# JosephCatrambone/aruco3

Measured on AMD Instinct MI355X. Metric: frames/sec at 1920x1080 ARUCO dict, higher is better.
Workload: dtype u8

## Files before the change

### aruco3_amd/_lib.py

```python
import ctypes as C
from pathlib import Path

import numpy as np

import os

_HERE = Path(__file__).resolve().parent
LIB_PATH = Path(os.environ["A3_HIP_LIB"]).resolve() if os.environ.get("A3_HIP_LIB") else _HERE / "libaruco3_hip.so"

OK, ERR_INVALID, ERR_HIP, ERR_CAPACITY, ERR_INTERNAL, ERR_NO_DEVICE, ERR_LIMIT = 0, -1, -2, -3, -4, -5, -6
FMT_RGB8, FMT_RGBA8, FMT_L8, FMT_BGRA8 = 0, 1, 2, 3
FMT_YUYV8, FMT_UYVY8 = 5, 6
MEM_HOST, MEM_DEVICE = 0, 1
PROFILE_OFF, PROFILE_STAGES, PROFILE_THRESHOLD_ONLY, PROFILE_THRESHOLD_SAMPLED = 0, 1, 2, 3
STAGE_THRESHOLD, STAGE_CONTOUR, STAGE_DECODE = 0, 1, 2
STEP_WHOLE, STEP_DECODE_DEFERRED, STEP_HELD_RELEASED_BY_LAST, STEP_HELD_RELEASED_EARLY, STEP_BURST_LAST, STEP_HELD = 0, 1, 2, 3, 4, 5
REFINE_NONE, REFINE_SUBPIX, REFINE_EDGES = 0, 1, 2
BOARD_NONE, BOARD_OK = 0, 1
BOARD_MAX_MARKERS = 1024
DIST_NONE, DIST_RATIONAL = 0, 1
DIST_FISHEYE = 3
CHARUCO_MAX_CORNERS = 2048
CHARUCO_NO_ADJ = 0xFFFFFFFF
CALIB_FIX_PRINCIPAL_POINT, CALIB_ZERO_TANGENT_DIST, CALIB_FIX_K3, CALIB_RATIONAL_MODEL, CALIB_USE_INTRINSIC_GUESS = 1, 2, 4, 8, 16
# ... 27 lines not shown
    "a3_candidate_count", "a3_download_candidates", "a3_download_homographies", "a3_estimate_pose", "a3_estimate_pose_normalized",
    "a3_find_nearest", "a3_calculate_tau", "a3_set_profiling", "a3_get_profile",
    "a3_contour_count", "a3_download_contours", "a3_detection_record_bytes", "a3_pack_detections",
    "a3_default_refine_config", "a3_set_corner_refinement", "a3_get_refined_corners", "a3_refine_corners",
    "a3_set_board", "a3_get_board_poses", "a3_estimate_board_pose",
    "a3_default_recover_config", "a3_set_board_recovery", "a3_get_board_recovery", "a3_get_recovered_counts", "a3_recover_markers",
    "a3_default_distortion", "a3_set_distortion", "a3_get_undistorted_corners", "a3_undistort_points",
    "a3_default_charuco_config", "a3_set_charuco", "a3_get_charuco_corners", "a3_get_charuco_poses", "a3_interpolate_charuco",
    "a3_calibrate_cameras", "a3_calibrate_fisheye_cameras", "a3_calibrate_rigs", "a3_calibrate_hand_eyes", "a3_build_marker_maps",
    "a3_default_rectify", "a3_rectify_frames", "a3_set_rectification", "a3_get_rectification",
    "a3_reduce_frames", "a3_set_reduction", "a3_get_reduction",
]
CAND_DTYPE = np.dtype([("start_key", "<u4"), ("xy", "<u2", (8,))])
PROJ_DTYPE = np.dtype([("inv", "<f4", (9,)), ("ok", "<i4")])
CONTOUR_DTYPE = np.dtype([("frame", "<u4"), ("start_key", "<u4"), ("point_base", "<u4"), ("n", "<u4")])
INTERNAL_SYMBOLS = ["a3_debug_set_overlap", "a3_debug_build_flags", "a3_debug_spin", "a3_debug_set_hold", "a3_debug_set_jump_rounds", "a3_debug_launch_threshold", "a3_debug_kernel_time", "a3_selftest_ieee", "a3_debug_clockwise", "a3_debug_rotate_bits", "a3_debug_discard_too_near", "a3_debug_inject_candidates", "a3_debug_sample_frames", "a3_debug_frame_candidates", "a3_debug_contour_quads"]


class A3Error(RuntimeError):
    def __init__(self, code, message):
        super().__init__(f"aruco3_hip error {code}: {message}")
        self.code = code


class Config(C.Structure):
    _fields_ = [
        ("threshold_window", C.c_uint32),
        ("contour_simplification_epsilon", C.c_double),
        ("min_side_length_factor", C.c_float),
        ("min_corner_separation_factor", C.c_float),
        ("homography_sample_size", C.c_uint32),
# ... 180 lines not shown


class RectifyInfo(C.Structure):
    _fields_ = [("tiles", C.c_uint32), ("path_tiles", C.c_uint32 * 4), ("reserved", C.c_uint32 * 3)]


class Stats(C.Structure):
    _fields_ = [("darts", C.c_uint64), ("contours_traced", C.c_uint64), ("contours_materialised", C.c_uint64),
                ("candidates_pre", C.c_uint64), ("candidates", C.c_uint64), ("markers", C.c_uint64),
                ("resolve_iterations", C.c_uint32), ("jump_rounds", C.c_uint32), ("chunks", C.c_uint32), ("stepping", C.c_uint32)]

    def as_dict(self):
        d = {k: int(getattr(self, k)) for k, _ in self._fields_}
        d["released_others"] = (d["stepping"] >> 8) & 0xFF
        d["reruns"] = (d["stepping"] >> 16) & 0xFF
        d["stepping"] = STEP_NAMES.get(d["stepping"] & 0xFF, d["stepping"] & 0xFF)
        return d


_lib = None


def load():
    global _lib
    if _lib is not None:
        return _lib
    try:
        import torch
    except ImportError:
        pass
# ... 49 lines not shown
    L.a3_synth_render.restype = C.c_int
    L.a3_synth_render.argtypes = [C.c_int, vp, vp, C.c_uint32, vp, C.c_uint32, C.c_uint32, C.c_uint32, C.c_int, C.c_float, C.c_float, C.c_int,
                                  vp, C.c_size_t, C.c_size_t]
    if hasattr(L, "a3_debug_set_overlap"):
        L.a3_debug_set_overlap.restype = C.c_int
        L.a3_debug_set_overlap.argtypes = [C.c_int]
    if hasattr(L, "a3_debug_launch_threshold"):
        L.a3_debug_launch_threshold.restype = C.c_int
        L.a3_debug_launch_threshold.argtypes = [vp, vp, C.c_int, C.c_uint32, C.c_uint32, C.c_uint32]
    if hasattr(L, "a3_debug_set_hold"):
        L.a3_debug_set_hold.restype = C.c_int
        L.a3_debug_set_hold.argtypes = [C.c_int]
    if hasattr(L, "a3_debug_set_jump_rounds"):
        L.a3_debug_set_jump_rounds.restype = C.c_int
        L.a3_debug_set_jump_rounds.argtypes = [C.c_int]
    if hasattr(L, "a3_debug_spin"):
        L.a3_debug_spin.restype = C.c_int
        L.a3_debug_spin.argtypes = [vp, C.c_int, C.c_int, C.c_int]
    if hasattr(L, "a3_debug_build_flags"):
        L.a3_debug_build_flags.restype = C.c_int
        L.a3_debug_build_flags.argtypes = []
    L.a3_debug_kernel_time.restype = C.c_int
    L.a3_debug_kernel_time.argtypes = [vp, C.c_int, C.c_int, C.c_int, C.POINTER(C.c_float)]
    L.a3_get_stats.restype = C.c_int
    L.a3_get_stats.argtypes = [vp, C.POINTER(Stats)]
    L.a3_download_grey.restype = C.c_int
    L.a3_download_grey.argtypes = [vp, C.c_uint32, u8p]
    L.a3_download_thresholded.restype = C.c_int
    L.a3_download_thresholded.argtypes = [vp, C.c_uint32, u8p]
    L.a3_candidate_count.restype = C.c_int
# ... 280 lines not shown
        check(load().a3_set_profiling(self.handle, int(mode)), self.handle)

    def profile(self, stage: int, reset: bool = False):
        ms, n = C.c_double(), C.c_uint64()
        check(load().a3_get_profile(self.handle, stage, C.byref(ms), C.byref(n), int(reset)), self.handle)
        return float(ms.value), int(n.value)

    def debug_kernel_time(self, kernel: int, dbg: int = 0, reps: int = 5) -> float:
        ms = C.c_float()
        check(load().a3_debug_kernel_time(self.handle, kernel, dbg, reps, C.byref(ms)), self.handle)
        return ms.value

    def stats(self) -> dict:
        s = Stats()
        check(load().a3_get_stats(self.handle, C.byref(s)), self.handle)
        return s.as_dict()

    def detect_batch(self, pixels_ptr: int, memory: int, fmt: int, width: int, height: int, row_stride: int, frame_stride: int, n_frames: int,
                     out_cap: int = 0):
        cap = out_cap or max(64 * n_frames, 64)
        out = np.empty(cap, dtype=MARKER_DTYPE)
        per = np.zeros(max(n_frames, 1), dtype=np.uint32)
        n = C.c_size_t()
        rc = load().a3_detect_batch(self.handle, C.c_void_p(pixels_ptr), memory, fmt, width, height, row_stride, frame_stride, n_frames,
                                    out.ctypes.data_as(C.c_void_p), cap, _p(per, C.c_uint32), C.byref(n))
        check(rc, self.handle)
        return out[: n.value], per[:n_frames]

    def submit(self, pixels_ptr: int, memory: int, fmt: int, width: int, height: int, row_stride: int, frame_stride: int, n_frames: int,
               out_cap: int = 0):
        self._pending = (out_cap or max(64 * n_frames, 64), n_frames)
# ... 432 lines not shown
```

### aruco3_amd/csrc/a3_api.hip

```cpp
#include <algorithm>
#include <atomic>
#include <cmath>
#include <chrono>
#include <cstddef>
#include <cstdio>
#include <cstring>
#include <mutex>
#include <string>
#include <vector>

#include "a3_common.h"
#include "a3_format.h"
#include "a3_internal.h"
#include "a3_launch.h"
#include "a3_readback.h"
#include "a3_rectify_check.h"
#include "a3_reduce_check.h"
#include "a3_solve_check.h"

using namespace a3;

namespace {

thread_local std::string g_create_error;
// ... 60 lines not shown
    uint32_t frames_W = 0, frames_H = 0;
    a3_rectify rect_r{};
    uint32_t reduce_f = 0;
    bool taps = false;
    bool sample_frames = false;
    int profiling = 0, profile_every = 1;
    int prof = 0;
    bool need_grey = false;
    bool grey_src = false;
    uint32_t max_cand = 0, patch_cap = 0, marker_cap = 0, guess = 0;
    bool active = false, device_plan = false;
    size_t n_chunks = 0;
    Readback rb;
    uint64_t chunk0_darts = 0;
    int rounds_max = 0;
    PixelSrc src{};
};

}

struct a3_ctx {
    int device = 0;
    hipStream_t own_stream = nullptr, stream = nullptr;
    hipEvent_t ev_in = nullptr;
    hipEvent_t ev_contours = nullptr, ev_k1 = nullptr, ev_k1_done = nullptr, ev_gate = nullptr;
    bool gates_declared = false;
    bool rest_held = false;
    int held_rc = 0;
    bool back_deferred = false;
    int back_rc = 0;
    bool allow_defer = false;
    int batch_mode = 0;
    std::atomic<uint32_t> stepping{0};
    uint32_t released_others = 0;
    uint32_t reruns = 0;
    a3_config cfg{};
    uint8_t num_bits = 0, tau = 0;
    uint32_t n_codes = 0, mark_size = 0;
    std::string err;

    uint64_t max_darts = kMaxDartsDefault;
    BatchHints hints;
    uint32_t dbg_nd = 0, dbg_frames = 0, dbg_chunks = 0;
    PixelSrc dbg_src{};
    std::vector<CandRec> inject;
    bool inject_armed = false;
    uint32_t inject_count = 0;
    Batch batch;
    bool pending_trivial = false;
// ... 138 lines not shown
    A3_HIP(ctx->t_cur.ensure(darts * 8));
    A3_HIP(ctx->t_next.ensure(darts * 8));
    A3_HIP(ctx->leader_list.ensure(leader_list_bytes((uint32_t)darts)));
    A3_HIP(ctx->leader_keep.ensure(leader_list_bytes((uint32_t)darts)));
    const size_t eslots = entry_slots((uint32_t)darts);
    A3_HIP(ctx->entry_list.ensure(eslots * 4));
    A3_HIP(ctx->es_a.ensure(eslots * entry_state_bytes()));
    A3_HIP(ctx->es_b.ensure(eslots * entry_state_bytes()));
    return A3_OK;
}

struct DeviceStreams { hipStream_t decode = nullptr, copy = nullptr; };
std::mutex g_streams_mu;
DeviceStreams g_dev_streams[64];
bool g_hold_rests = true;
std::atomic<int> g_jump_rounds_cap{0};
enum { kStreamCopy = 0, kStreamDecode = 1 };

hipError_t create_stream(hipStream_t* st) { return hipStreamCreateWithPriority(st, hipStreamNonBlocking, 0); }

hipError_t device_stream(int device, int kind, hipStream_t* out) {
    std::lock_guard<std::mutex> lk(g_streams_mu);
    DeviceStreams& ds = g_dev_streams[device & 63];
    hipStream_t& st = kind == kStreamDecode ? ds.decode : ds.copy;
    if (!st) {
        const hipError_t e = create_stream(&st);
        if (e != hipSuccess) { st = nullptr; return e; }
    }
    *out = st;
    return hipSuccess;
// ... 300 lines not shown
                                      .bits = ctx->bin.as<uint64_t>(), .hsum_tmp = big_window ? ctx->hsum.as<uint16_t>() : nullptr}));
    if (b.prof) A3_HIP(hipEventRecord(ctx->ev[1], st));
    if (!held) return A3_OK;
    A3_HIP(hipEventRecord(ctx->ev_k1_done, st));
    const uint64_t cap_d = device_plan_capacity(ctx->hints, ctx->max_darts, n, W, H);
    if (cap_d == 0) return fail(ctx, A3_ERR_INTERNAL, "a chain was held back for a batch that needs a host-side plan");
    return ensure_chain_buffers(ctx, st, b, cap_d);
}

ContourChunk contour_chunk(const a3_ctx* ctx) {
    ContourChunk c;
    c.W = (int)ctx->W; c.H = (int)ctx->H; c.batch_frames = ctx->frames;
    c.bits = ctx->bin.as<uint64_t>(); c.tile_darts = ctx->tile_darts.as<uint32_t>(); c.pix_base = ctx->pix_base.as<uint32_t>();
    c.d_rec = ctx->d_xy.as<uint64_t>(); c.d_succ = ctx->d_succ.as<uint32_t>();
    c.entry_list = ctx->entry_list.as<uint32_t>(); c.es_a = ctx->es_a.p; c.es_b = ctx->es_b.p; c.fin = ctx->fin.p;
    c.leader_count = ctx->head->leader_count; c.entry_count = ctx->head->entry_count;
    c.leader_list = ctx->leader_list.as<uint32_t>(); c.leader_keep = ctx->leader_keep.as<uint32_t>();
    c.t_cur = ctx->t_cur.as<uint64_t>(); c.t_next = ctx->t_next.as<uint64_t>();
    c.contours = ctx->contours.as<ContourRec>(); c.cyc_start_off = ctx->cyc_start_off.as<uint32_t>(); c.points = ctx->points.as<uint32_t>();
    c.max_contours = ctx->hints.max_contours; c.max_points = ctx->hints.max_points;
    c.cands = ctx->cands.as<CandRec>(); c.cand_count = ctx->cand_count;
    c.err_flags = &ctx->head->err_flags;
    return c;
}

int enqueue_chain(a3_ctx* ctx, Batch& b, bool defer_locked) {
    hipStream_t st = ctx->stream;
    const uint32_t n = b.n, W = b.W, H = b.H;
    const int rel_mode = defer_locked ? 0 : release_mode();
    const size_t npx = (size_t)W * H;
    const uint32_t minwh = W < H ? W : H;
// ... 77 lines not shown
        uint32_t* h_bases = reinterpret_cast<uint32_t*>((uint8_t*)ctx->pinned + (size_t)n * 8);
        for (size_t ci = 0; ci < chunks.size(); ci++) chunk_frame_bases(fd.data(), chunks[ci], (uint32_t)stride, h_bases + ci * stride);
        A3_HIP(hipMemcpyAsync(ctx->frame_base.p, h_bases, n_bases * 4, hipMemcpyHostToDevice, st));
    }
    ctx->stats.chunks = (uint32_t)chunks.size();

    ContourChunk cc = contour_chunk(ctx);
    cc.n_live = n_live;
    cc.resolve_iters = ctx->hints.resolve_full_ttl > 0 ? ctx->hints.resolve_iters_hint : 0;
    cc.inline_resolve_W = ctx->hints.resolve_full_ttl > 0 ? 0 : (int)W;
    cc.min_edge_length = min_edge_length;
    cc.eps_factor = ctx->cfg.contour_simplification_epsilon;
    cc.keep_all = b.taps;
    cc.max_cand = kMaxCand;
    int rounds_max = 0;
    for (size_t ci = 0; ci < chunks.size(); ci++) {
        const Chunk& c = chunks[ci];
        const uint32_t nd = (uint32_t)c.darts;
        if (nd == 0) continue;
        if (ci > 0) {
            A3_HIP(hipMemsetAsync(cc.leader_count, 0, sizeof(BatchScratch::leader_count) + sizeof(BatchScratch::entry_count), st));
            A3_HIP(hipMemsetAsync(ctx->frame_cursor, 0, (size_t)c.count * 4, st));
        }
        cc.first_frame = c.first; cc.n_frames = c.count; cc.n_darts = nd;
        cc.frame_base = ctx->frame_base.as<uint32_t>() + ci * (max_chunk_frames + 1);
        cc.ctr = ctx->counters + ci;
        A3_HIP(launch_dart_build(st, cc));
        const int rounds = chunk_rounds(c.max_frame_darts, ctx->hints.jump_rounds_hint, g_jump_rounds_cap.load(std::memory_order_relaxed));
        rounds_max = std::max(rounds_max, rounds);
        cc.max_rounds = rounds;
        cc.frame_entries = ctx->hints.entry_global_ttl > 0 ? nullptr : ctx->frame_cursor;
        const bool dense_graph = (uint64_t)nd * 10u >= (uint64_t)c.count * npx;
        cc.dead_count = (b.taps || !dense_graph) ? nullptr : ctx->head->dead_count;
        cc.phase = 1;
        A3_HIP(launch_rank_cycles(st, cc));
        if (rel_mode == 2) { if (int rc = release_waiting()) return rc; }
        ctx->dbg_nd = nd; ctx->dbg_frames = c.count; ctx->dbg_chunks = (uint32_t)chunks.size();
        cc.phase = 2;
        A3_HIP(launch_rank_cycles(st, cc));
        A3_HIP(launch_resolve(st, cc));
        A3_HIP(launch_select_scatter(st, cc));
        A3_HIP(launch_contour_quads(st, cc));
    }
    if (rel_mode != 0) { if (int rc = release_waiting()) return rc; }
    if (b.prof >= 2) A3_HIP(hipEventRecord(ctx->ev[2], st));

// ... 34 lines not shown
    hipStream_t st = ctx->stream;
    const size_t n_chunks = b.n_chunks;
    const uint32_t guess = b.guess, n = b.n;
    uint8_t* hp = (uint8_t*)ctx->pinned;
    Readback rb = b.rb;
    {
        std::lock_guard<std::mutex> lk(g_defer_mu);
        if (int rc = flush_deferred_locked(ctx, nullptr)) return rc;
        if (const int rc = ctx->back_rc) { ctx->back_rc = 0; return rc; }
    }
    A3_HIP(wait_event(ctx->ev[4], st));
    const BatchScratch& hs = *reinterpret_cast<const BatchScratch*>(hp);
    const DeviceCounters* hc = reinterpret_cast<const DeviceCounters*>(&hs + 1);
    const size_t slot_bytes = sizeof(CandRec) + 16 + 16 + 4 + decode_out_bytes() + proj_rec_bytes();
    const Verdict v = batch_verdict(hs, hc, {.n = n, .W = b.W, .H = b.H, .device_plan = b.device_plan, .n_chunks = n_chunks, .chunk0_darts = b.chunk0_darts,
                                             .rounds_max = b.rounds_max, .out_cap = out_cap, .lds_slots = frame_cand_lds_slots(), .slot_bytes = slot_bytes},
                                    ctx->hints);
    if (b.device_plan && !hs.plan.overflow) ctx->stats.darts = ctx->dbg_nd = v.darts;
    ctx->stats.contours_traced = v.contours_traced; ctx->stats.contours_materialised = v.contours_materialised;
    ctx->stats.jump_rounds = v.jump_rounds; ctx->stats.resolve_iterations = v.resolve_iterations;
    if (v.action == Verdict::Fail) return fail(ctx, v.code, v.message);
    if (v.action == Verdict::GrowCands) {
        const size_t had = ctx->cands.cap + ctx->pre_xy.cap + ctx->fin_xy.cap + ctx->work.cap + ctx->cand_big.cap + ctx->outs.cap + ctx->proj.cap;
        const size_t want = (size_t)n * v.next_cand * v.slot_bytes;
        size_t free_b = 0, total_b = 0;
        if (want > had && hipMemGetInfo(&free_b, &total_b) == hipSuccess && want - had > free_b)
            return fail(ctx, A3_ERR_LIMIT, "candidate tables of this batch do not fit the device (every frame gets the fullest frame's table): fewer frames per call");
        ctx->hints.max_cand = v.next_cand;
    }
    if (v.action != Verdict::Deliver) return 1;
    const uint32_t total = v.total, n_work = v.n_work, n_pre = v.n_pre;
    const uint32_t* hpf = reinterpret_cast<const uint32_t*>(hc + n_chunks);
    if (per_frame_count) memcpy(per_frame_count, hpf, (size_t)n * 4);
    uint32_t max_per_frame = 0;
    for (uint32_t f = 0; f < n; f++) max_per_frame = std::max(max_per_frame, hpf[f]);
// ... 423 lines not shown
    const int rc = stage_input(ctx, pixels, memory, fmt, width, height, &b.row_stride, &b.frame_stride, n_frames, &b.pixels);
    if (rc != A3_OK) return rc;
    b.frames = PixelSrc{b.pixels, b.row_stride, b.frame_stride, fmt}; b.frames_W = width; b.frames_H = height;
    b.plane = ctx->rect_on ? Batch::Plane::Rectified : ctx->reduction.factor ? Batch::Plane::Reduced : Batch::Plane::None;
    if (b.plane != Batch::Plane::None) {
        size_t w, h;
        if (b.plane == Batch::Plane::Rectified) { b.rect_r = ctx->rect; w = b.rect_r.dst.image_width; h = b.rect_r.dst.image_height; }
        else { b.reduce_f = ctx->reduction.factor; w = width / b.reduce_f; h = height / b.reduce_f; }
        A3_HIP(ctx->plane.ensure(w * h * n_frames));
        b.pixels = ctx->plane.as<uint8_t>(); b.fmt = A3_FMT_L8; b.W = (uint32_t)w; b.H = (uint32_t)h;
        b.row_stride = w; b.frame_stride = w * h;
    }
    if (b.board || b.charuco || b.recover) { if (int urc = upload_board(ctx)) return urc; }
    if (b.recover) { if (int urc = upload_recover_ids(ctx)) return urc; }
    if (b.charuco) { if (int urc = upload_charuco(ctx)) return urc; }
    ctx->hints.force_host_plan = false;
    ctx->reruns = 0; ctx->released_others = 0;
    return A3_OK;
}

static void finish_trivial(a3_ctx* ctx, uint32_t* per_frame_count) {
    const Batch& b = ctx->batch;
    if (per_frame_count && b.n) memset(per_frame_count, 0, (size_t)b.n * 4);
    for (int k = 0; k < kSideKinds; k++) {
        if (!kSides[k].kept) continue;
        ctx->side_h[k].assign(b.has(k) && kSides[k].per_frame ? b.n * kSides[k].rec : 0, 0);
        ctx->side_valid[k] = b.has(k);
    }
    ctx->h_charuco.clear(); ctx->charuco_valid = b.charuco;
}

static int run_batch_with_retries(a3_ctx* ctx, a3_marker* out, a3_pose* poses, size_t out_cap, uint32_t* per_frame_count, size_t* out_n) {
// ... 219 lines not shown
}

int a3_debug_set_hold(int on) {
    std::lock_guard<std::mutex> lk(g_defer_mu);
    if (!g_held.empty()) return A3_ERR_INVALID;
    g_hold_rests = on != 0;
    return A3_OK;
}

int a3_debug_set_jump_rounds(int rounds) {
    if (rounds < 0 || rounds > 32) return A3_ERR_INVALID;
    g_jump_rounds_cap.store(rounds, std::memory_order_relaxed);
    return A3_OK;
}

int a3_synth_render(int device, void* hip_stream, const a3_synth_frame* frames, uint32_t n_frames, const a3_synth_marker* markers,
                    uint32_t n_markers, uint32_t width, uint32_t height, int paper, float black, float white, int supersample,
                    void* out_rgb_device, size_t row_stride, size_t frame_stride) {
    if (!frames || !out_rgb_device || (n_markers && !markers) || supersample < 1 || supersample > 8) return A3_ERR_INVALID;
    if (n_frames == 0 || width == 0 || height == 0) return A3_OK;
    if (row_stride == 0) row_stride = (size_t)width * 3;
    if (frame_stride == 0) frame_stride = row_stride * height;
    if (row_stride < (size_t)width * 3 || frame_stride < row_stride * (height - 1) + (size_t)width * 3 || height > 65535 || n_frames > 65535)
        return A3_ERR_INVALID;
    for (uint32_t f = 0; f < n_frames; f++)
        if ((uint64_t)frames[f].first_marker + frames[f].n_markers > n_markers) return A3_ERR_INVALID;
    for (uint32_t m = 0; m < n_markers; m++)
        if (markers[m].n == 0 || markers[m].n > 11) return A3_ERR_INVALID;
    if (hipSetDevice(device) != hipSuccess) return A3_ERR_NO_DEVICE;
    hipStream_t st = reinterpret_cast<hipStream_t>(hip_stream);
// ... 2 lines not shown
    if (e == hipSuccess && n_markers) e = hipMalloc(&d_markers, sizeof(a3_synth_marker) * n_markers);
    if (e == hipSuccess) e = hipMemcpyAsync(d_frames, frames, sizeof(a3_synth_frame) * n_frames, hipMemcpyHostToDevice, st);
    if (e == hipSuccess && n_markers) e = hipMemcpyAsync(d_markers, markers, sizeof(a3_synth_marker) * n_markers, hipMemcpyHostToDevice, st);
    if (e == hipSuccess) e = launch_synth_render(st, {.frames = d_frames, .n_frames = n_frames, .markers = d_markers, .W = width, .H = height, .paper = paper,
                                                      .black = black, .white = white, .supersample = supersample,
                                                      .out = reinterpret_cast<uint8_t*>(out_rgb_device), .row_stride = row_stride, .frame_stride = frame_stride});
    if (e == hipSuccess) e = hipStreamSynchronize(st);
    if (d_frames) (void)hipFree(d_frames);
    if (d_markers) (void)hipFree(d_markers);
    return e == hipSuccess ? A3_OK : A3_ERR_HIP;
}

int a3_get_stats(const a3_ctx* ctx, a3_stats* stats) {
    if (!ctx || !stats) return A3_ERR_INVALID;
    *stats = ctx->stats;
    stats->stepping = ctx->stepping | (std::min(ctx->released_others, 255u) << 8) | (std::min(ctx->reruns, 255u) << 16);
    return A3_OK;
}

static int download_plane(a3_ctx* ctx, const DevBuf& buf, uint32_t frame, uint8_t* dst) {
    if (!ctx || !dst) return A3_ERR_INVALID;
    if (frame >= ctx->frames) return fail(ctx, A3_ERR_INVALID, "frame index outside the last batch");
    const size_t npx = (size_t)ctx->W * ctx->H;
    A3_HIP(hipSetDevice(ctx->device));
    if (int rcs_ = need_stream(ctx)) return rcs_;
    A3_HIP(hipMemcpy(dst, buf.as<uint8_t>() + npx * frame, npx, hipMemcpyDeviceToHost));
    return A3_OK;
}

int a3_download_grey(a3_ctx* ctx, uint32_t frame, uint8_t* dst) {
    if (!ctx) return A3_ERR_INVALID;
// ... 1139 lines not shown
```

### aruco3_amd/csrc/a3_batch_head.h

```cpp
#pragma once
#include <cstddef>
#include <cstdint>

#include "../../include/aruco3_hip.h"

namespace a3 {

template <typename T> constexpr T min_of(T a, T b) { return b < a ? b : a; }
template <typename T> constexpr T max_of(T a, T b) { return a < b ? b : a; }

constexpr uint32_t kMaxChunkFrames = 65536u;
constexpr int kResolveItersMax = 16;
constexpr uint32_t kLeaderShards = 16, kEntryShards = 16, kDeadShards = 16;

struct DeviceCounters {
    unsigned long long darts;
    unsigned long long points;
    unsigned int contours;
    unsigned int traced;
    unsigned int err_flags;
    unsigned int resolve_needed;
    unsigned int jump_changed[32];
    unsigned int resolve_changed[16];
    unsigned int entry_overflow;
    unsigned int pad[1];
};
static_assert(sizeof(DeviceCounters::resolve_changed) / sizeof(unsigned int) == kResolveItersMax, "one resolve_changed slot per pass");

constexpr unsigned kErrBrokenEvent = 1u,
                   kErrPointPool = 2u, kErrContourTable = 4u, kErrCandTable = 8u,
                   kErrResolve = 16u,
                   kErrMarkerCap = 32u,
                   kErrScatter = 64u;

struct PlanWords {
    uint32_t darts;
    uint32_t overflow;
    uint32_t max_frame_darts;
    uint32_t total_clamped;
};
struct BatchScratch {
    unsigned int work_count;
    unsigned int marker_total;
    unsigned int cand_pre_total;
    unsigned int pack_overflow;
    unsigned int err_flags;
    unsigned int cand_most;
    unsigned int unused6[2];
    PlanWords plan;
    unsigned int unused12[4];
    unsigned int leader_count[kLeaderShards];
    unsigned int entry_count[kEntryShards];
    unsigned int dead_count[kDeadShards];
};
static_assert(offsetof(BatchScratch, work_count) == 0 && offsetof(BatchScratch, marker_total) == 4 && offsetof(BatchScratch, cand_pre_total) == 8 &&
              offsetof(BatchScratch, pack_overflow) == 12 && offsetof(BatchScratch, err_flags) == 16 && offsetof(BatchScratch, cand_most) == 20 &&
              offsetof(BatchScratch, plan) == 32 && offsetof(PlanWords, darts) == 0 && offsetof(PlanWords, overflow) == 4 &&
              offsetof(PlanWords, max_frame_darts) == 8 && offsetof(PlanWords, total_clamped) == 12 && offsetof(BatchScratch, leader_count) == 64 &&
              offsetof(BatchScratch, entry_count) == 128 && offsetof(BatchScratch, dead_count) == 192 && sizeof(BatchScratch) == 256,
              "the scratch words' offsets are part of the read-back head");
static_assert(offsetof(BatchScratch, entry_count) == offsetof(BatchScratch, leader_count) + sizeof(BatchScratch::leader_count),
              "leader and entry counts are cleared by one memset");
constexpr unsigned kCandMostFromPre = (offsetof(BatchScratch, cand_most) - offsetof(BatchScratch, cand_pre_total)) / sizeof(unsigned int);

constexpr uint32_t kMaxCandDefault = 1024, kMaxCandLimit = A3_MAX_CANDIDATES_PER_FRAME;
static_assert(kMaxCandLimit == 65536, "a3_marker.candidate_index is a uint16_t");
constexpr uint32_t kMaxContoursDefault = 1u << 20;
constexpr uint64_t kMaxDartsDefault = 48ull << 20;
constexpr uint64_t kMaxPointsDefault = 64ull << 20;
constexpr uint64_t kHardMaxDarts = (1ull << 30) - (1ull << 16);
constexpr uint64_t kHardMaxPoints = 3ull << 30;

struct BatchHints {
    int jump_rounds_hint = 10, resolve_iters_hint = 4;
    int resolve_full_ttl = 0;
    int entry_global_ttl = 0;
    bool plan_valid = false, force_host_plan = false;
    uint32_t plan_n = 0, plan_W = 0, plan_H = 0;
    uint64_t plan_darts = 0;
    uint64_t max_points = kMaxPointsDefault;
    uint32_t max_contours = kMaxContoursDefault;
    uint32_t max_cand = kMaxCandDefault;
};

struct BatchFacts {
    uint32_t n, W, H; bool device_plan; size_t n_chunks; uint64_t chunk0_darts; int rounds_max; size_t out_cap; uint32_t lds_slots; size_t slot_bytes;
};
struct Verdict {
    enum Action { Deliver, Rerun, GrowCands, Fail } action = Deliver;
    int code = A3_OK; const char* message = nullptr;
    uint32_t next_cand = 0; size_t slot_bytes = 0;
    uint64_t darts = 0, contours_traced = 0, contours_materialised = 0; uint32_t jump_rounds = 0, resolve_iterations = 0;
    uint32_t total = 0, n_work = 0, n_pre = 0;
    uint32_t tap_contours = 0; uint64_t tap_points = 0;
};

inline Verdict batch_verdict(const BatchScratch& hs, const DeviceCounters* hc, const BatchFacts& f, BatchHints& h) {
    Verdict v;
    const auto rerun = [&v]() { v.action = Verdict::Rerun; return v; };
    const auto fail = [&v](int code, const char* message) { v.action = Verdict::Fail; v.code = code; v.message = message; return v; };
    if (f.device_plan) {
        if (hs.plan.overflow) { h.force_host_plan = true; return rerun(); }
        v.darts = hs.plan.darts;
        h.plan_darts = hs.plan.darts;
    } else {
        h.plan_valid = f.n_chunks == 1;
        h.plan_n = f.n; h.plan_W = f.W; h.plan_H = f.H;
        h.plan_darts = f.n_chunks == 1 ? f.chunk0_darts : 0;
    }
    unsigned int flags = hs.err_flags;
    for (unsigned int dead : hs.dead_count) v.contours_traced += dead;
    uint64_t need_points = 0; uint32_t need_contours = 0;
    bool jump_short = false, resolve_needed = false, entry_overflow = false;
    for (size_t ci = 0; ci < f.n_chunks; ci++) {
        const DeviceCounters& c = hc[ci];
        flags |= c.err_flags;
        resolve_needed |= c.resolve_needed != 0;
        entry_overflow |= c.entry_overflow != 0;
        need_points = max_of<uint64_t>(need_points, c.points);
        need_contours = max_of(need_contours, c.contours);
        v.contours_traced += c.traced;
        v.contours_materialised += c.contours;
        for (int r = 0; r < 32; r++) if (c.jump_changed[r]) v.jump_rounds = max_of<uint32_t>(v.jump_rounds, r + 1);
        uint32_t it = c.resolve_needed ? 1 : 0;
        for (int r = 0; r < kResolveItersMax - 1; r++) if (c.resolve_changed[r]) it = r + 2;
        v.resolve_iterations = max_of(v.resolve_iterations, it);
        if (f.rounds_max > 0 && f.rounds_max < 32 && c.jump_changed[f.rounds_max - 1] != 0) jump_short = true;
    }
    if (entry_overflow) { h.entry_global_ttl = 64; h.jump_rounds_hint = max_of(h.jump_rounds_hint, 12); return rerun(); }
    if (h.entry_global_ttl > 0) h.entry_global_ttl--;
    if (jump_short && h.jump_rounds_hint < 32) { h.jump_rounds_hint = 32; return rerun(); }
    if (resolve_needed) {
        const bool ran = h.resolve_full_ttl > 0;
        h.resolve_full_ttl = 64;
        if (!ran) return rerun();
    } else if (h.resolve_full_ttl > 0) h.resolve_full_ttl--;
    if ((flags & kErrResolve) && h.resolve_iters_hint < kResolveItersMax) { h.resolve_iters_hint = kResolveItersMax; return rerun(); }
    h.jump_rounds_hint = max_of(4, min_of(32, (int)v.jump_rounds + 2));
    if (flags & (kErrPointPool | kErrContourTable)) {
        if (need_points > h.max_points) h.max_points = min_of<uint64_t>(kHardMaxPoints, max_of(need_points, h.max_points * 2));
        if (need_contours > h.max_contours) h.max_contours = max_of(need_contours, h.max_contours * 2);
        return rerun();
    }
    if (flags & kErrBrokenEvent) return fail(A3_ERR_INTERNAL, "contour graph: a start event lies on an open chain");
// ... 91 lines not shown
```

### aruco3_amd/csrc/a3_internal.h

```cpp
#ifndef ARUCO3_HIP_INTERNAL_H
#define ARUCO3_HIP_INTERNAL_H

#include "../../include/aruco3_hip.h"

#ifdef __cplusplus
extern "C" {
#endif

int  a3_debug_kernel_time(a3_ctx *ctx, int kernel, int dbg, int reps, float *avg_ms);

int  a3_debug_set_overlap(int mode);

int  a3_debug_spin(void *hip_stream, int workgroups, int threads, int usec);

int  a3_debug_set_hold(int on);

int  a3_debug_set_jump_rounds(int rounds);

int  a3_debug_launch_threshold(a3_ctx *ctx, const void *pixels_device, int fmt, uint32_t width, uint32_t height, uint32_t n_frames);

int  a3_debug_build_flags(void);

int  a3_selftest_ieee(a3_ctx *ctx, const double *a, const double *b, size_t n, double *sqrt_a, double *a_div_b,
                      float *sqrtf_a, float *a_divf_b);

int  a3_debug_clockwise(a3_ctx *ctx, const int32_t *quads_xy, size_t n, int32_t *out_xy);
int  a3_debug_rotate_bits(a3_ctx *ctx, const uint8_t *bits, uint32_t n, uint32_t times, uint8_t *out);
int  a3_debug_inject_candidates(a3_ctx *ctx, const uint32_t *quads_xy, size_t n);
int  a3_debug_sample_frames(a3_ctx *ctx, int enabled);
int  a3_debug_discard_too_near(a3_ctx *ctx, const uint32_t *quads_xy, size_t n, float min_distance, uint32_t *out_xy, size_t *n_out);

typedef struct { uint32_t start_key; uint16_t xy[8]; } a3_debug_cand;
// ... 16 lines not shown
```

### aruco3_amd/csrc/a3_launch.h

```cpp
#pragma once

#include "a3_common.h"

namespace a3 {

struct ThresholdLaunch {
    const uint8_t* pixels = nullptr; int fmt = 0; size_t row_stride = 0, frame_stride = 0; int W = 0, H = 0; uint32_t n = 0, radius = 0;
    uint8_t* grey = nullptr; uint64_t* bits = nullptr; uint16_t* hsum_tmp = nullptr;
};
hipError_t launch_grey_threshold(hipStream_t st, const ThresholdLaunch& t);
bool threshold_writes_grey_plane(uint32_t radius);
hipError_t launch_k1_r1(hipStream_t st, const ThresholdLaunch& t);
hipError_t launch_k1_r2(hipStream_t st, const ThresholdLaunch& t);
bool ring_kernel_applies(uint32_t radius);
hipError_t launch_ring_threshold(hipStream_t st, const ThresholdLaunch& t);

size_t tile_darts_bytes(uint32_t W, uint32_t H, uint32_t n_frames);
struct DartCountLaunch {
    const uint64_t* bits = nullptr; int W = 0, H = 0; uint32_t first_frame = 0, n_frames = 0; unsigned long long* frame_darts = nullptr;
    uint32_t* tile_darts = nullptr; uint64_t plan_cap = 0; uint32_t* frame_base = nullptr; PlanWords* plan = nullptr; void* zero_p = nullptr;
    size_t zero_bytes = 0;
};
hipError_t launch_dart_count(hipStream_t st, const DartCountLaunch& d);
hipError_t launch_zero(hipStream_t st, void* p, size_t bytes);

size_t entry_state_bytes();
size_t fin_state_bytes();
size_t entry_slots(uint32_t n_darts);
size_t leader_list_bytes(uint32_t n_darts);

struct ContourChunk {
    uint32_t first_frame = 0, n_frames = 0, n_darts = 0; const uint32_t* frame_base = nullptr; DeviceCounters* ctr = nullptr;
    int max_rounds = 0;
    uint32_t* frame_entries = nullptr;
    unsigned int* dead_count = nullptr;
    int W = 0, H = 0;
    uint32_t batch_frames = 0;
    const uint64_t* bits = nullptr; const uint32_t* tile_darts = nullptr;
    const uint32_t* n_live = nullptr;
    uint32_t* pix_base = nullptr; uint64_t* d_rec = nullptr; uint32_t* d_succ = nullptr; uint32_t* entry_list = nullptr;
    unsigned int* entry_count = nullptr, * leader_count = nullptr;
    void* es_a = nullptr, * es_b = nullptr;
    void* fin = nullptr;
    uint32_t* leader_list = nullptr, * leader_keep = nullptr; uint64_t* t_cur = nullptr, * t_next = nullptr;
    int resolve_iters = 0;
    int inline_resolve_W = 0;
    uint32_t min_edge_length = 0; double eps_factor = 0.0; ContourRec* contours = nullptr; uint32_t* cyc_start_off = nullptr;
    uint32_t* points = nullptr; uint32_t max_contours = 0; uint64_t max_points = 0;
    bool keep_all = false;
// ... 167 lines not shown
```

### aruco3_amd/csrc/k_contours.hip

```cpp
#include <algorithm>
#include <cmath>

#include "a3_common.h"
#include "a3_launch.h"


namespace a3 {

constexpr int kFinB = 8;
constexpr int kScatB = 1;

struct Nb8 { uint64_t c; uint64_t n[8]; };

__device__ __forceinline__ uint64_t ldw(const uint64_t* __restrict__ img, int wpr, int H, int j, int y) {
    return (y >= 0 && y < H && j >= 0 && j < wpr) ? img[(size_t)y * wpr + j] : 0ull;
}

__device__ __forceinline__ void pdart_words(const Nb8& nb, uint64_t p[8]) {
#pragma unroll
    for (int k = 0; k < 8; k++) {
        uint64_t m = nb.c & nb.n[k] & ~nb.n[(k + 7) & 7];
        if ((k & 1) == 0) m &= ~nb.n[(k + 6) & 7];
        p[k] = m;
    }
// ... 800 lines not shown
        const uint32_t excl = block_excl_scan_256((uint32_t)__popc(lmask), s_lw, &total);
        if (total) {
            const uint32_t shard = blockIdx.x & (kLeaderShards - 1);
            if (threadIdx.x == 0) s_lbase = atomicAdd(&leader_count[shard], total);
            __syncthreads();
            uint32_t slot = s_lbase + excl;
            while (lmask) {
                const int u = __ffs(lmask) - 1;
                lmask &= lmask - 1;
                leader_list[(size_t)shard * leader_cap + slot++] = lo + threadIdx.x + (uint32_t)u * 256u;
            }
        }
    }
}

constexpr uint32_t kEntryLdsCap = 2048;
__global__ __launch_bounds__(256) void k_entry_frame(const uint32_t* __restrict__ entry_list, const uint32_t* __restrict__ frame_entries,
                                                     const uint32_t* __restrict__ frame_base, const FinState* __restrict__ fin,
                                                     const uint64_t* __restrict__ d_rec, int W,
                                                     EntryState* __restrict__ es, DeviceCounters* __restrict__ ctr,
                                                     uint32_t* __restrict__ leader_list ,
                                                     unsigned int* __restrict__ leader_count , uint32_t leader_cap) {
    struct __attribute__((aligned(16))) Rec { uint64_t key; uint32_t ptr; uint32_t off; };
    __shared__ Rec s_rec[kEntryLdsCap];
    __shared__ uint32_t s_dist[kEntryLdsCap];
    const uint32_t f = blockIdx.x;
    const uint32_t cnt = frame_entries[f], base = frame_base[f];
    if (cnt == 0) return;
    if (cnt > kEntryLdsCap) { if (threadIdx.x == 0) ctr->entry_overflow = 1u; return; }
    constexpr int PER = kEntryLdsCap / 256;
    uint64_t nk[PER]; uint32_t np[PER], no[PER], nd[PER];
    uint32_t m0[PER];
    constexpr int EB = 4;
    static_assert(PER % EB == 0, "whole batches");
#pragma unroll
    for (int u0 = 0; u0 < PER; u0 += EB) {
        if ((uint32_t)u0 * 256u >= cnt) break;
        uint32_t e[EB];
        FinState l[EB];
        uint64_t mr[EB];
#pragma unroll
        for (int u = 0; u < EB; u++) e[u] = entry_list[base + min(threadIdx.x + 256u * (uint32_t)(u0 + u), cnt - 1u)];
#pragma unroll
        for (int u = 0; u < EB; u++) l[u] = fin[e[u]];
#pragma unroll
        for (int u = 0; u < EB; u++) mr[u] = d_rec[entry_min_dart(e[u], l[u])];
#pragma unroll
        for (int u = 0; u < EB; u++) asm volatile("" : "+v"(mr[u]), "+v"(l[u].leader), "+v"(l[u].w));
#pragma unroll
        for (int u = 0; u < EB; u++) {
            const uint32_t i = threadIdx.x + 256u * (uint32_t)(u0 + u);
            const EntryState s0 = entry_start(e[u], l[u], mr[u], W, base + i);
            nk[u0 + u] = s0.key; no[u0 + u] = s0.off; nd[u0 + u] = s0.dist; np[u0 + u] = s0.ptr - base; m0[u0 + u] = (uint32_t)s0.key;
            if (i < cnt) { s_rec[i] = Rec{nk[u0 + u], np[u0 + u], no[u0 + u]}; s_dist[i] = nd[u0 + u]; }
        }
    }
    __syncthreads();
    for (int round = 0; round < 12; round++) {
        int changed = 0;
#pragma unroll
        for (int u = 0; u < PER; u++) {
            const uint32_t i = threadIdx.x + u * 256;
            if (i < cnt) {
                const uint32_t t = np[u] < cnt ? np[u] : i;
                const Rec w = s_rec[t];
                const uint32_t wd = s_dist[t];
                if (w.key < nk[u]) { nk[u] = w.key; no[u] = nd[u] + w.off; changed = 1; }
                nd[u] += wd;
                np[u] = w.ptr;
            }
        }
        const int any = __syncthreads_or(changed);
#pragma unroll
// ... 674 lines not shown
                               entry_list, entry_count, ecap, frame_base, frame_entries, n_live, dbg, min_edge_length, dead_count, trust_natural,
                               ll, leader_count, lcap);
        else if (frame_entries)
            hipLaunchKernelGGL((k_local_contract<kLTFrame, true>), dim3((n_darts + kLTFrame - 1) / kLTFrame), dim3(256), 0, st, n_darts, W, d_rec, d_succ, fin,
                               entry_list, entry_count, ecap, frame_base, frame_entries, n_live, dbg, min_edge_length, dead_count, trust_natural,
                               ll, leader_count, lcap);
        else
            hipLaunchKernelGGL((k_local_contract<kLT, true>), dim3((n_darts + kLT - 1) / kLT), dim3(256), 0, st, n_darts, W, d_rec, d_succ, fin,
                               entry_list, entry_count, ecap, frame_base, frame_entries, n_live, dbg, min_edge_length, dead_count, trust_natural,
                               ll, leader_count, lcap);
    }
    if (dbg || phase == 1) return hipGetLastError();
    EntryState* a = reinterpret_cast<EntryState*>(c.es_a);
    EntryState* b = reinterpret_cast<EntryState*>(c.es_b);
    if (frame_entries) {
        hipLaunchKernelGGL(k_entry_frame, dim3(n_frames), dim3(256), 0, st, entry_list, frame_entries, frame_base, fin, d_rec, W, a, ctr,
                           ll, leader_count, lcap);
        if (no_finalize) return hipGetLastError();
        const int fin_blocks = std::max(blocks_for(n_darts, 256, kFinBlocks), (int)(((uint64_t)n_darts + 256ull * 32 - 1) / (256ull * 32)));
        hipLaunchKernelGGL(k_jump_finalize, dim3(fin_blocks), dim3(256), 0, st, n_darts, a, fin,
                           leader_list, leader_count, leader_shard_cap(n_darts), n_live, ctr);
        return hipGetLastError();
    }
    const dim3 grid(blocks_for(n_darts / 16 + 1, 256, 1024)), block(256);
    hipLaunchKernelGGL(k_entry_init, grid, block, 0, st, entry_list, entry_count, fin, d_rec, W, a, ecap);
    for (int r = 0; r < c.max_rounds; r++) {
        hipLaunchKernelGGL(k_entry_jump, grid, block, 0, st, a, b, entry_count, ecap, r, ctr);
        EntryState* t = a; a = b; b = t;
    }
    const int fin_blocks = std::max(blocks_for(n_darts, 256, kFinBlocks), (int)(((uint64_t)n_darts + 256ull * 32 - 1) / (256ull * 32)));
    hipLaunchKernelGGL(k_jump_finalize, dim3(fin_blocks), block, 0, st, n_darts, a, fin,
                       leader_list, leader_count, leader_shard_cap(n_darts), n_live, ctr);
// ... 58 lines not shown
```

Before: 374,400.

## Template per-frame entry kernel on adaptive LDS capacity with rerun on overflow

The per-frame entry pointer-jumping kernel is templated on its LDS capacity (512, 1024 or 2048 entries). The host picks the capacity from a hint that tracks the largest per-frame entry count seen, and reruns the batch at a larger capacity when a frame does not fit. Smaller capacities use less LDS and fewer registers per thread, and need fewer jump rounds (10 or 11 instead of 12), which should raise occupancy and cut work. The cost is an extra atomicMax per block, added host hint logic, and possible full-batch reruns when entry counts grow past the chosen cap.

```diff
diff --git a/aruco3_amd/_lib.py b/aruco3_amd/_lib.py
--- a/aruco3_amd/_lib.py
+++ b/aruco3_amd/_lib.py
@@ -65,7 +65,7 @@
 CAND_DTYPE = np.dtype([("start_key", "<u4"), ("xy", "<u2", (8,))])
 PROJ_DTYPE = np.dtype([("inv", "<f4", (9,)), ("ok", "<i4")])
 CONTOUR_DTYPE = np.dtype([("frame", "<u4"), ("start_key", "<u4"), ("point_base", "<u4"), ("n", "<u4")])
-INTERNAL_SYMBOLS = ["a3_debug_set_overlap", "a3_debug_build_flags", "a3_debug_spin", "a3_debug_set_hold", "a3_debug_set_jump_rounds", "a3_debug_launch_threshold", "a3_debug_kernel_time", "a3_selftest_ieee", "a3_debug_clockwise", "a3_debug_rotate_bits", "a3_debug_discard_too_near", "a3_debug_inject_candidates", "a3_debug_sample_frames", "a3_debug_frame_candidates", "a3_debug_contour_quads"]
+INTERNAL_SYMBOLS = ["a3_debug_set_overlap", "a3_debug_build_flags", "a3_debug_spin", "a3_debug_set_hold", "a3_debug_set_jump_rounds", "a3_debug_set_entry_cap", "a3_debug_entry_info", "a3_debug_launch_threshold", "a3_debug_kernel_time", "a3_selftest_ieee", "a3_debug_clockwise", "a3_debug_rotate_bits", "a3_debug_discard_too_near", "a3_debug_inject_candidates", "a3_debug_sample_frames", "a3_debug_frame_candidates", "a3_debug_contour_quads"]
 
 
 class A3Error(RuntimeError):
@@ -276,6 +276,7 @@
         d = {k: int(getattr(self, k)) for k, _ in self._fields_}
         d["released_others"] = (d["stepping"] >> 8) & 0xFF
         d["reruns"] = (d["stepping"] >> 16) & 0xFF
+        d["entry_cap"] = ((d["stepping"] >> 24) & 0xFF) * 256
         d["stepping"] = STEP_NAMES.get(d["stepping"] & 0xFF, d["stepping"] & 0xFF)
         return d
 
@@ -355,6 +356,11 @@
     if hasattr(L, "a3_debug_set_jump_rounds"):
         L.a3_debug_set_jump_rounds.restype = C.c_int
         L.a3_debug_set_jump_rounds.argtypes = [C.c_int]
+    if hasattr(L, "a3_debug_set_entry_cap"):
+        L.a3_debug_set_entry_cap.restype = C.c_int
+        L.a3_debug_set_entry_cap.argtypes = [C.c_uint32]
+        L.a3_debug_entry_info.restype = C.c_int
+        L.a3_debug_entry_info.argtypes = [vp, C.POINTER(C.c_uint32), C.POINTER(C.c_uint32)]
     if hasattr(L, "a3_debug_spin"):
         L.a3_debug_spin.restype = C.c_int
         L.a3_debug_spin.argtypes = [vp, C.c_int, C.c_int, C.c_int]
@@ -665,7 +671,12 @@
     def stats(self) -> dict:
         s = Stats()
         check(load().a3_get_stats(self.handle, C.byref(s)), self.handle)
-        return s.as_dict()
+        d = s.as_dict()
+        if hasattr(load(), "a3_debug_entry_info"):
+            most, short = C.c_uint32(0), C.c_uint32(0)
+            check(load().a3_debug_entry_info(self.handle, C.byref(most), C.byref(short)), self.handle)
+            d["entry_most"], d["entry_cap_reruns"] = most.value, short.value
+        return d
 
     def detect_batch(self, pixels_ptr: int, memory: int, fmt: int, width: int, height: int, row_stride: int, frame_stride: int, n_frames: int,
                      out_cap: int = 0):
diff --git a/aruco3_amd/csrc/a3_api.hip b/aruco3_amd/csrc/a3_api.hip
--- a/aruco3_amd/csrc/a3_api.hip
+++ b/aruco3_amd/csrc/a3_api.hip
@@ -98,6 +98,7 @@
     Readback rb;
     uint64_t chunk0_darts = 0;
     int rounds_max = 0;
+    uint32_t entry_cap = 0;
     PixelSrc src{};
 };
 
@@ -117,6 +118,7 @@
     int batch_mode = 0;
     std::atomic<uint32_t> stepping{0};
     uint32_t released_others = 0;
+    uint32_t entry_cap = 0, entry_most = 0, entry_cap_reruns = 0;
     uint32_t reruns = 0;
     a3_config cfg{};
     uint8_t num_bits = 0, tau = 0;
@@ -285,6 +287,7 @@
 std::mutex g_streams_mu;
 DeviceStreams g_dev_streams[64];
 bool g_hold_rests = true;
+std::atomic<uint32_t> g_entry_cap_force{0};
 std::atomic<int> g_jump_rounds_cap{0};
 enum { kStreamCopy = 0, kStreamDecode = 1 };
 
@@ -615,7 +618,7 @@
     c.bits = ctx->bin.as<uint64_t>(); c.tile_darts = ctx->tile_darts.as<uint32_t>(); c.pix_base = ctx->pix_base.as<uint32_t>();
     c.d_rec = ctx->d_xy.as<uint64_t>(); c.d_succ = ctx->d_succ.as<uint32_t>();
     c.entry_list = ctx->entry_list.as<uint32_t>(); c.es_a = ctx->es_a.p; c.es_b = ctx->es_b.p; c.fin = ctx->fin.p;
-    c.leader_count = ctx->head->leader_count; c.entry_count = ctx->head->entry_count;
+    c.leader_count = ctx->head->leader_count; c.entry_count = ctx->head->entry_count; c.entry_most = &ctx->head->entry_most;
     c.leader_list = ctx->leader_list.as<uint32_t>(); c.leader_keep = ctx->leader_keep.as<uint32_t>();
     c.t_cur = ctx->t_cur.as<uint64_t>(); c.t_next = ctx->t_next.as<uint64_t>();
     c.contours = ctx->contours.as<ContourRec>(); c.cyc_start_off = ctx->cyc_start_off.as<uint32_t>(); c.points = ctx->points.as<uint32_t>();
@@ -723,6 +726,9 @@
     cc.keep_all = b.taps;
     cc.max_cand = kMaxCand;
     int rounds_max = 0;
+    const uint32_t entry_force = ctx->hints.entry_cap_retry ? 0u : g_entry_cap_force.load(std::memory_order_relaxed);
+    cc.entry_cap = entry_force ? entry_force : entry_cap_of(ctx->hints.entry_most_hint);
+    b.entry_cap = 0;
     for (size_t ci = 0; ci < chunks.size(); ci++) {
         const Chunk& c = chunks[ci];
         const uint32_t nd = (uint32_t)c.darts;
@@ -739,6 +745,7 @@
         rounds_max = std::max(rounds_max, rounds);
         cc.max_rounds = rounds;
         cc.frame_entries = ctx->hints.entry_global_ttl > 0 ? nullptr : ctx->frame_cursor;
+        if (cc.frame_entries) b.entry_cap = cc.entry_cap;
         const bool dense_graph = (uint64_t)nd * 10u >= (uint64_t)c.count * npx;
         cc.dead_count = (b.taps || !dense_graph) ? nullptr : ctx->head->dead_count;
         cc.phase = 1;
@@ -803,11 +810,13 @@
     const DeviceCounters* hc = reinterpret_cast<const DeviceCounters*>(&hs + 1);
     const size_t slot_bytes = sizeof(CandRec) + 16 + 16 + 4 + decode_out_bytes() + proj_rec_bytes();
     const Verdict v = batch_verdict(hs, hc, {.n = n, .W = b.W, .H = b.H, .device_plan = b.device_plan, .n_chunks = n_chunks, .chunk0_darts = b.chunk0_darts,
-                                             .rounds_max = b.rounds_max, .out_cap = out_cap, .lds_slots = frame_cand_lds_slots(), .slot_bytes = slot_bytes},
+                                             .rounds_max = b.rounds_max, .out_cap = out_cap, .lds_slots = frame_cand_lds_slots(), .slot_bytes = slot_bytes, .entry_cap = b.entry_cap},
                                     ctx->hints);
     if (b.device_plan && !hs.plan.overflow) ctx->stats.darts = ctx->dbg_nd = v.darts;
     ctx->stats.contours_traced = v.contours_traced; ctx->stats.contours_materialised = v.contours_materialised;
     ctx->stats.jump_rounds = v.jump_rounds; ctx->stats.resolve_iterations = v.resolve_iterations;
+    ctx->entry_cap = b.entry_cap; ctx->entry_most = std::max(ctx->entry_most, v.entry_most);
+    if (v.entry_cap_short) ctx->entry_cap_reruns++;
     if (v.action == Verdict::Fail) return fail(ctx, v.code, v.message);
     if (v.action == Verdict::GrowCands) {
         const size_t had = ctx->cands.cap + ctx->pre_xy.cap + ctx->fin_xy.cap + ctx->work.cap + ctx->cand_big.cap + ctx->outs.cap + ctx->proj.cap;
@@ -1261,8 +1270,8 @@
     if (b.board || b.charuco || b.recover) { if (int urc = upload_board(ctx)) return urc; }
     if (b.recover) { if (int urc = upload_recover_ids(ctx)) return urc; }
     if (b.charuco) { if (int urc = upload_charuco(ctx)) return urc; }
-    ctx->hints.force_host_plan = false;
-    ctx->reruns = 0; ctx->released_others = 0;
+    ctx->hints.force_host_plan = false; ctx->hints.entry_cap_retry = false;
+    ctx->reruns = 0; ctx->released_others = 0; ctx->entry_cap_reruns = 0; ctx->entry_most = 0;
     return A3_OK;
 }
 
@@ -1512,6 +1521,18 @@
     return A3_OK;
 }
 
+int a3_debug_set_entry_cap(uint32_t cap) {
+    if (cap != 0 && cap != 512 && cap != 1024 && cap != 2048) return A3_ERR_INVALID;
+    g_entry_cap_force.store(cap, std::memory_order_relaxed);
+    return A3_OK;
+}
+
+int a3_debug_entry_info(const a3_ctx* ctx, uint32_t* most, uint32_t* cap_reruns) {
+    if (!ctx || !most || !cap_reruns) return A3_ERR_INVALID;
+    *most = ctx->entry_most; *cap_reruns = ctx->entry_cap_reruns;
+    return A3_OK;
+}
+
 int a3_synth_render(int device, void* hip_stream, const a3_synth_frame* frames, uint32_t n_frames, const a3_synth_marker* markers,
                     uint32_t n_markers, uint32_t width, uint32_t height, int paper, float black, float white, int supersample,
                     void* out_rgb_device, size_t row_stride, size_t frame_stride) {
@@ -1544,7 +1565,7 @@
 int a3_get_stats(const a3_ctx* ctx, a3_stats* stats) {
     if (!ctx || !stats) return A3_ERR_INVALID;
     *stats = ctx->stats;
-    stats->stepping = ctx->stepping | (std::min(ctx->released_others, 255u) << 8) | (std::min(ctx->reruns, 255u) << 16);
+    stats->stepping = ctx->stepping | (std::min(ctx->released_others, 255u) << 8) | (std::min(ctx->reruns, 255u) << 16) | ((ctx->entry_cap / 256u) << 24);
     return A3_OK;
 }
 
diff --git a/aruco3_amd/csrc/a3_batch_head.h b/aruco3_amd/csrc/a3_batch_head.h
--- a/aruco3_amd/csrc/a3_batch_head.h
+++ b/aruco3_amd/csrc/a3_batch_head.h
@@ -25,6 +25,7 @@
     unsigned int entry_overflow;
     unsigned int pad[1];
 };
+constexpr unsigned kEntryOverflow = 1u, kEntryCapShort = 2u;
 static_assert(sizeof(DeviceCounters::resolve_changed) / sizeof(unsigned int) == kResolveItersMax, "one resolve_changed slot per pass");
 
 constexpr unsigned kErrBrokenEvent = 1u,
@@ -46,7 +47,8 @@
     unsigned int pack_overflow;
     unsigned int err_flags;
     unsigned int cand_most;
-    unsigned int unused6[2];
+    unsigned int entry_most;
+    unsigned int unused7[1];
     PlanWords plan;
     unsigned int unused12[4];
     unsigned int leader_count[kLeaderShards];
@@ -54,7 +56,7 @@
     unsigned int dead_count[kDeadShards];
 };
 static_assert(offsetof(BatchScratch, work_count) == 0 && offsetof(BatchScratch, marker_total) == 4 && offsetof(BatchScratch, cand_pre_total) == 8 &&
-              offsetof(BatchScratch, pack_overflow) == 12 && offsetof(BatchScratch, err_flags) == 16 && offsetof(BatchScratch, cand_most) == 20 &&
+              offsetof(BatchScratch, pack_overflow) == 12 && offsetof(BatchScratch, err_flags) == 16 && offsetof(BatchScratch, cand_most) == 20 && offsetof(BatchScratch, entry_most) == 24 &&
               offsetof(BatchScratch, plan) == 32 && offsetof(PlanWords, darts) == 0 && offsetof(PlanWords, overflow) == 4 &&
               offsetof(PlanWords, max_frame_darts) == 8 && offsetof(PlanWords, total_clamped) == 12 && offsetof(BatchScratch, leader_count) == 64 &&
               offsetof(BatchScratch, entry_count) == 128 && offsetof(BatchScratch, dead_count) == 192 && sizeof(BatchScratch) == 256,
@@ -75,6 +77,8 @@
     int jump_rounds_hint = 10, resolve_iters_hint = 4;
     int resolve_full_ttl = 0;
     int entry_global_ttl = 0;
+    uint32_t entry_most_hint = 0;
+    bool entry_cap_retry = false;
     bool plan_valid = false, force_host_plan = false;
     uint32_t plan_n = 0, plan_W = 0, plan_H = 0;
     uint64_t plan_darts = 0;
@@ -83,8 +87,21 @@
     uint32_t max_cand = kMaxCandDefault;
 };
 
+constexpr uint32_t kEntryCapMin = 512, kEntryCapMax = 2048;
+inline uint32_t entry_cap_of(uint32_t hint) { return hint == 0 ? kEntryCapMax : hint <= 512 ? 512u : hint <= 1024 ? 1024u : kEntryCapMax; }
+inline uint32_t entry_hint_follow(uint32_t hint, uint32_t most) {
+    const uint32_t want = max_of(kEntryCapMin, min_of<uint32_t>(kEntryCapMax, most <= kEntryCapMax / 2 ? most * 2u : kEntryCapMax));
+    if (hint == 0) return want;
+    hint = max_of(kEntryCapMin, min_of(kEntryCapMax, hint));
+    return want >= hint ? want : max_of(want, hint - hint / 8u);
+}
+inline uint32_t entry_hint_grow(uint32_t cap, uint32_t most) {
+    return max_of(min_of(kEntryCapMax, max_of(cap, kEntryCapMin / 2) * 2u), entry_hint_follow(kEntryCapMin, most));
+}
+
 struct BatchFacts {
     uint32_t n, W, H; bool device_plan; size_t n_chunks; uint64_t chunk0_darts; int rounds_max; size_t out_cap; uint32_t lds_slots; size_t slot_bytes;
+    uint32_t entry_cap = 0;
 };
 struct Verdict {
     enum Action { Deliver, Rerun, GrowCands, Fail } action = Deliver;
@@ -93,6 +110,8 @@
     uint64_t darts = 0, contours_traced = 0, contours_materialised = 0; uint32_t jump_rounds = 0, resolve_iterations = 0;
     uint32_t total = 0, n_work = 0, n_pre = 0;
     uint32_t tap_contours = 0; uint64_t tap_points = 0;
+    uint32_t entry_most = 0;
+    bool entry_cap_short = false;
 };
 
 inline Verdict batch_verdict(const BatchScratch& hs, const DeviceCounters* hc, const BatchFacts& f, BatchHints& h) {
@@ -111,12 +130,13 @@
     unsigned int flags = hs.err_flags;
     for (unsigned int dead : hs.dead_count) v.contours_traced += dead;
     uint64_t need_points = 0; uint32_t need_contours = 0;
-    bool jump_short = false, resolve_needed = false, entry_overflow = false;
+    bool jump_short = false, resolve_needed = false, entry_overflow = false, entry_cap_short = false;
     for (size_t ci = 0; ci < f.n_chunks; ci++) {
         const DeviceCounters& c = hc[ci];
         flags |= c.err_flags;
         resolve_needed |= c.resolve_needed != 0;
-        entry_overflow |= c.entry_overflow != 0;
+        entry_overflow |= (c.entry_overflow & ~kEntryCapShort) != 0;
+        entry_cap_short |= (c.entry_overflow & kEntryCapShort) != 0;
         need_points = max_of<uint64_t>(need_points, c.points);
         need_contours = max_of(need_contours, c.contours);
         v.contours_traced += c.traced;
@@ -127,7 +147,17 @@
         v.resolve_iterations = max_of(v.resolve_iterations, it);
         if (f.rounds_max > 0 && f.rounds_max < 32 && c.jump_changed[f.rounds_max - 1] != 0) jump_short = true;
     }
-    if (entry_overflow) { h.entry_global_ttl = 64; h.jump_rounds_hint = max_of(h.jump_rounds_hint, 12); return rerun(); }
+    if (f.entry_cap) v.entry_most = hs.entry_most;
+    if (entry_overflow) {
+        h.entry_global_ttl = 64; h.jump_rounds_hint = max_of(h.jump_rounds_hint, 12); h.entry_most_hint = kEntryCapMax; h.entry_cap_retry = false;
+        return rerun();
+    }
+    if (entry_cap_short) {
+        h.entry_most_hint = entry_hint_grow(f.entry_cap, v.entry_most); h.entry_cap_retry = true; v.entry_cap_short = true;
+        return rerun();
+    }
+    h.entry_cap_retry = false;
+    if (f.entry_cap) h.entry_most_hint = entry_hint_follow(h.entry_most_hint, v.entry_most);
     if (h.entry_global_ttl > 0) h.entry_global_ttl--;
     if (jump_short && h.jump_rounds_hint < 32) { h.jump_rounds_hint = 32; return rerun(); }
     if (resolve_needed) {
diff --git a/aruco3_amd/csrc/a3_internal.h b/aruco3_amd/csrc/a3_internal.h
--- a/aruco3_amd/csrc/a3_internal.h
+++ b/aruco3_amd/csrc/a3_internal.h
@@ -16,6 +16,9 @@
 int  a3_debug_set_hold(int on);
 
 int  a3_debug_set_jump_rounds(int rounds);
+
+int  a3_debug_set_entry_cap(uint32_t cap);
+int  a3_debug_entry_info(const a3_ctx *ctx, uint32_t *most, uint32_t *cap_reruns);
 
 int  a3_debug_launch_threshold(a3_ctx *ctx, const void *pixels_device, int fmt, uint32_t width, uint32_t height, uint32_t n_frames);
 
diff --git a/aruco3_amd/csrc/a3_launch.h b/aruco3_amd/csrc/a3_launch.h
--- a/aruco3_amd/csrc/a3_launch.h
+++ b/aruco3_amd/csrc/a3_launch.h
@@ -33,6 +33,8 @@
     uint32_t first_frame = 0, n_frames = 0, n_darts = 0; const uint32_t* frame_base = nullptr; DeviceCounters* ctr = nullptr;
     int max_rounds = 0;
     uint32_t* frame_entries = nullptr;
+    uint32_t entry_cap = kEntryCapMax;
+    unsigned int* entry_most = nullptr;
     unsigned int* dead_count = nullptr;
     int W = 0, H = 0;
     uint32_t batch_frames = 0;
diff --git a/aruco3_amd/csrc/k_contours.hip b/aruco3_amd/csrc/k_contours.hip
--- a/aruco3_amd/csrc/k_contours.hip
+++ b/aruco3_amd/csrc/k_contours.hip
@@ -838,24 +838,28 @@
     }
 }
 
-constexpr uint32_t kEntryLdsCap = 2048;
+constexpr uint32_t kEntryLdsCap = kEntryCapMax;
+template <uint32_t CAP>
 __global__ __launch_bounds__(256) void k_entry_frame(const uint32_t* __restrict__ entry_list, const uint32_t* __restrict__ frame_entries,
                                                      const uint32_t* __restrict__ frame_base, const FinState* __restrict__ fin,
                                                      const uint64_t* __restrict__ d_rec, int W,
                                                      EntryState* __restrict__ es, DeviceCounters* __restrict__ ctr,
                                                      uint32_t* __restrict__ leader_list ,
-                                                     unsigned int* __restrict__ leader_count , uint32_t leader_cap) {
+                                                     unsigned int* __restrict__ leader_count , uint32_t leader_cap,
+                                                     unsigned int* __restrict__ entry_most ) {
+    static_assert(CAP >= 512 && CAP <= kEntryLdsCap && (CAP & (CAP - 1)) == 0, "512, 1024 or 2048");
     struct __attribute__((aligned(16))) Rec { uint64_t key; uint32_t ptr; uint32_t off; };
-    __shared__ Rec s_rec[kEntryLdsCap];
-    __shared__ uint32_t s_dist[kEntryLdsCap];
+    __shared__ Rec s_rec[CAP];
+    __shared__ uint32_t s_dist[CAP];
     const uint32_t f = blockIdx.x;
     const uint32_t cnt = frame_entries[f], base = frame_base[f];
     if (cnt == 0) return;
-    if (cnt > kEntryLdsCap) { if (threadIdx.x == 0) ctr->entry_overflow = 1u; return; }
-    constexpr int PER = kEntryLdsCap / 256;
+    if (threadIdx.x == 0 && entry_most) atomicMax(entry_most, cnt);
+    if (cnt > CAP) { if (threadIdx.x == 0) atomicOr(&ctr->entry_overflow, cnt > kEntryLdsCap ? kEntryOverflow : kEntryCapShort); return; }
+    constexpr int PER = CAP / 256;
     uint64_t nk[PER]; uint32_t np[PER], no[PER], nd[PER];
     uint32_t m0[PER];
-    constexpr int EB = 4;
+    constexpr int EB = PER < 4 ? PER : 4;
     static_assert(PER % EB == 0, "whole batches");
 #pragma unroll
     for (int u0 = 0; u0 < PER; u0 += EB) {
@@ -880,7 +884,8 @@
         }
     }
     __syncthreads();
-    for (int round = 0; round < 12; round++) {
+    constexpr int kRounds = (CAP == 512 ? 9 : CAP == 1024 ? 10 : 11) + 1;
+    for (int round = 0; round < kRounds; round++) {
         int changed = 0;
 #pragma unroll
         for (int u = 0; u < PER; u++) {
@@ -1585,8 +1590,9 @@
     EntryState* a = reinterpret_cast<EntryState*>(c.es_a);
     EntryState* b = reinterpret_cast<EntryState*>(c.es_b);
     if (frame_entries) {
-        hipLaunchKernelGGL(k_entry_frame, dim3(n_frames), dim3(256), 0, st, entry_list, frame_entries, frame_base, fin, d_rec, W, a, ctr,
-                           ll, leader_count, lcap);
+        const auto entry_frame = c.entry_cap <= 512 ? k_entry_frame<512> : c.entry_cap <= 1024 ? k_entry_frame<1024> : k_entry_frame<kEntryLdsCap>;
+        hipLaunchKernelGGL(entry_frame, dim3(n_frames), dim3(256), 0, st, entry_list, frame_entries, frame_base, fin, d_rec, W, a, ctr,
+                           ll, leader_count, lcap, c.entry_most);
         if (no_finalize) return hipGetLastError();
         const int fin_blocks = std::max(blocks_for(n_darts, 256, kFinBlocks), (int)(((uint64_t)n_darts + 256ull * 32 - 1) / (256ull * 32)));
         hipLaunchKernelGGL(k_jump_finalize, dim3(fin_blocks), dim3(256), 0, st, n_darts, a, fin,
```

Measured after the change: 378,000, median of 3. About the same (+0.9%).
